# mpitid/babble

Hardware: AMD Instinct MI355X
Metric: consensus-ordered events/sec at N participants (higher is better)
Workload: dtype int32; 1 GPU; random-gossip DAG, 256 participants, 10000000 events per GPU, RunConsensus every K=256 events (39063 calls); participants=256, events_per_graph=10000000, k=256, graphs_per_gpu=1, parallelism=replicas1

## Files before the change

babble_amd/csrc/hge_engine.hip:

```cpp
#include <hip/hip_runtime.h>

#include <algorithm>
#include <chrono>
#include <cstdio>
#include <cstdlib>
#include <cstring>
#include <mutex>
#include <optional>
#include <string>
#include <thread>
#include <utility>
#include <vector>

#include "../../include/hge.h"
#include "hge_plan.h"
#include "hge_kernels.hip"
#include "hge_median_rows.hip"
#include "hge_wide32.hip"
#include "hge_coords.hip"
#include "hge_coords_win.hip"
#include "hge_rounds_coop.hip"
#include "hge_rounds_direct.hip"
#include "hge_walk_spec.hip"

// ... 1346 lines not shown
    if (getenv("HGE_WALK_DEBUG")) {
      std::vector<int32_t> hn(2 * nw);
      std::vector<uint64_t> mg(nw);
      readback(hn.data(), s_cn.p, hn.size());
      readback(mg.data(), s_cM.p, mg.size());
      fprintf(stderr, "coop walk: nw=%d Hcap=%d resume=%d |", nw, Hcap, hres[1]);
      for (int i = 0; i < nw; i++)
        fprintf(stderr, " %d:%d%s->(%d,w%d:%d)", i, hn[i], hn[nw + i] ? "e" : "",
                mg[i] == ~0ull ? -1 : (int)(mg[i] >> 32),
                mg[i] == ~0ull ? -1 : i + (int)((mg[i] >> 16) & 0xFFFF), (int)(mg[i] & 0xFFFF));
      fprintf(stderr, "\n");
    }
    return hres[1];
  }
  void wide_walk(Tables t, const CoordStep& s, int32_t rlo, const int32_t* rlo_dev, int Rprev) {
    const int32_t* FDT = d_FDT.p;
    const int32_t* olen = s.olen;
    const int32_t* len = s.len;
    int32_t* rstate = s.rstate;
    int32_t* err = s_bar.p + 1;
    uint64_t* gran = s_gran.p;
    uint64_t* ssc = d_ssc.p;
    uint64_t* dbg = dbg_p();
    if (direct_rounds()) {
      uint32_t* mb = walk_mb();
      unsigned long long* paths = walk_paths();
      unsigned long long* paths_next = s_wpaths.p + 2 * ((walk_seq + 1) & 1);
      const int32_t* nostart = nullptr;
      int32_t* nohist = nullptr;
      int hmax = 0, extra = 0;
      const char* hs = getenv("HGE_TEST_HANDOFF_STALL");
      int stall_ep = hs ? atoi(hs) : 0;
      int force_exact = walk_force_exact();
      void* dargs[] = {&t, &olen, &len, &rstate, &rlo, &rlo_dev, &Rprev, &gran, &err, &ssc, &mb, &dbg,
                       &nostart, &nohist, &hmax, &nostart, &extra, &stall_ep, &force_exact, &paths, &paths_next};
      prof_begin("k_rounds_direct");
      HIPCHK(launch_resident(direct_fn(), dim3(N), dim3(1024), dargs));
      prof_end();
    } else {
      void* args[] = {&t, &FDT, &olen, &len, &rstate, &rlo, &rlo_dev, &Rprev, &gran, &err, &ssc, &dbg};
      prof_begin("k_rounds_coop");
      HIPCHK(launch_resident((const void*)k_rounds_coop, dim3(N), dim3(COOP_BS), args));
      prof_end();
    }
    if (getenv("HGE_TEST_HANDOFF_FAIL")) {
      const int32_t one = 1, down = hge_plan::kRoundsStoodDown;
      h2d(err, &one, 4);
      h2d(rstate + 1, &down, 4);
    }
  }
  uint32_t* walk_mb() {
    s_mb.need((size_t)npow() * npow());
    return s_mb.p;
  }
  DBuf<unsigned long long> s_wpaths;
  int walk_seq = 0;
  unsigned long long* walk_paths() {
    if (!s_wpaths.p) {
      s_wpaths.need(4);
      HIPCHK(hipMemset(s_wpaths.p, 0, 4 * sizeof(unsigned long long)));
    }
    walk_seq++;
    return s_wpaths.p + 2 * (walk_seq & 1);
  }
  static int walk_force_exact() {
    const char* e = getenv("HGE_TEST_DIR_EXACT");
    return e && atoi(e) != 0 ? 1 : 0;
  }
  const void* direct_fn() const {
    return N <= 64 ? (const void*)k_rounds_direct<1024, 64>
         : N <= 128 ? (const void*)k_rounds_direct<1024, 128>
                    : (const void*)k_rounds_direct<1024, 256>;
  }

  bool sweep16() const { return N > 32 && !wide32; }
  bool wla16() const { return N > 192 && (N & 3) == 0 && !wide32; }

  void to_wide32() {
    auto test_stop = [&](int stage) {
      if (test_w32_fail == stage) {
        test_w32_fail = 0;
        throw EngineError(HGE_ERR_DEVICE, "test: to_wide32 stopped after stage " + std::to_string(stage));
      }
    };
    ensure_fdtd();
// ... 1575 lines not shown
  const int N = h->N, NW = h->NW;
  h->s_hist.need((size_t)hmax * N + N);
  h->s_hssc.need((size_t)hmax * N * NW);
  h->s_hstate.need(N + 4);
  h->h2d(h->s_hstate.p, start, 4 * (size_t)N);
  int32_t* cut = nullptr;
  if (stopcut) {
    h->s_hist.need((size_t)hmax * N + 2 * N);
    cut = h->s_hist.p + (size_t)hmax * N + N;
    h->h2d(cut, stopcut, 4 * (size_t)N);
  }
  int32_t* rstate = h->s_hstate.p + N;
  HIPCHK(hipMemsetAsync(rstate, 0, 16, h->st));
  h->s_bar.need(2);
  h->s_gran.need(2 * (size_t)N);
  HIPCHK(hipMemsetAsync(h->s_bar.p, 0, 8, h->st));
  HIPCHK(hipMemsetAsync(h->s_gran.p, 0, 16 * (size_t)N, h->st));
  auto lk = h->frontier_lock();
  Tables t = h->tables();
  const int32_t* olen = h->cstep->olen;
  const int32_t* len = h->cstep->len;
  int rlo = 0, Rprev = 0;
  const int32_t* rlo_dev = nullptr;
  uint64_t* gran = h->s_gran.p;
  int32_t* err = h->s_bar.p + 1;
  uint64_t* ssc = h->s_hssc.p;
  uint32_t* mb = h->walk_mb();
  unsigned long long* paths = h->walk_paths();
  unsigned long long* paths_next = h->s_wpaths.p + 2 * ((h->walk_seq + 1) & 1);
  uint64_t* dbg = nullptr;
  const int32_t* st0 = h->s_hstate.p;
  int32_t* hist = h->s_hist.p;
  int hm = hmax, ex = std::max(0, (int)extra), nostall = 0, force_exact = hge_engine::walk_force_exact();
  void* args[] = {&t, &olen, &len, &rstate, &rlo, &rlo_dev, &Rprev, &gran, &err, &ssc, &mb, &dbg,
                  &st0, &hist, &hm, &cut, &ex, &nostall, &force_exact, &paths, &paths_next};
  h->prof_begin("k_rounds_direct_walk");
  HIPCHK(h->launch_resident(h->direct_fn(), dim3(N), dim3(1024), args));
  h->prof_end();
  int32_t rs[2] = {0, 0}, e = 0;
  h->d2h(rs, rstate, 8);
  h->d2h(&e, err, 4);
  h->sync();
  if (e) throw EngineError(HGE_ERR_DEVICE, "rounds frontier hand-off timed out");
  const int n = std::max(1, std::min(rs[0], hmax));
  if (rows_out) h->readback(rows_out, h->s_hist.p, (size_t)n * N);
  if (ssc_out) h->readback(ssc_out, h->s_hssc.p, (size_t)n * N * NW);
  if (nrows) *nrows = n;
  if (natural) *natural = rs[1] == 0 ? 1 : 0;
  return HGE_OK;
  GUARD_END(h)
}

int hge_frontier_rows(hge_engine* h, int32_t from, int32_t n, int32_t* rows_out, uint64_t* ssc_out) {
  GUARD_BEGIN
  const int N = h->N, NW = h->NW;
  if (from < 0 || n < 0 || (size_t)(from + n) * N > h->s_hist.n) return HGE_ERR_ARG;
  if (rows_out && n) h->d2h(rows_out, h->s_hist.p + (size_t)from * N, 4 * (size_t)n * N);
  if (ssc_out && n) h->d2h(ssc_out, h->s_hssc.p + (size_t)from * N * NW, 8 * (size_t)n * N * NW);
  h->sync();
  return HGE_OK;
  GUARD_END(h)
}

int hge_split_finish(hge_engine* h, const int32_t* rows, const uint64_t* ssc, int32_t nrows,
                     int32_t natural, int64_t* n_ordered) {
  GUARD_BEGIN
  if (!h->cstep || !rows || nrows < 1 || (nrows > 1 && !ssc)) return HGE_ERR_ARG;
  const int N = h->N, NW = h->NW;
// ... 541 lines not shown
```

babble_amd/csrc/hge_narrow.h:

```cpp
#pragma once

#include <stdint.h>

#if defined(__HIPCC__) || defined(__CUDACC__)
#define HGE_NAR_HD __host__ __device__ __forceinline__
#else
#define HGE_NAR_HD inline
#endif

namespace hge_narrow {

constexpr uint32_t kNarGuard = 0x80808080u;
constexpr uint32_t kNarAMax = 126;
constexpr uint32_t kNarBaseNone = 0xFFFEu;
constexpr int32_t kNarBaseMax = 65400;
constexpr int32_t kNarInf32 = 0x7FFFFFFF;

HGE_NAR_HD uint32_t nar_base16(int32_t P) { return P == kNarInf32 ? kNarBaseNone : (uint32_t)P; }
HGE_NAR_HD bool nar_base_too_large(int32_t P) { return P != kNarInf32 && P > kNarBaseMax; }

HGE_NAR_HD uint32_t nar_sub_sat2(uint32_t x, uint32_t c) {
#if defined(__HIP_DEVICE_COMPILE__)
  typedef unsigned short u16x2 __attribute__((ext_vector_type(2)));
  const u16x2 r = __builtin_elementwise_sub_sat(__builtin_bit_cast(u16x2, x), __builtin_bit_cast(u16x2, c));
// ... 19 lines not shown
  const u16x2 r = __builtin_elementwise_max(__builtin_bit_cast(u16x2, x), __builtin_bit_cast(u16x2, y));
  return __builtin_bit_cast(uint32_t, r);
#else
  const uint32_t xl = x & 0xFFFFu, yl = y & 0xFFFFu, xh = x >> 16, yh = y >> 16;
  return (xl > yl ? xl : yl) | ((xh > yh ? xh : yh) << 16);
#endif
}
HGE_NAR_HD uint32_t nar_pack4(uint32_t x0, uint32_t x1) {
#if defined(__HIP_DEVICE_COMPILE__)
  return __builtin_amdgcn_perm(x1, x0, 0x06040200u);
#else
  return (x0 & 0xFFu) | ((x0 >> 8) & 0xFF00u) | ((x1 & 0xFFu) << 16) | ((x1 << 8) & 0xFF000000u);
#endif
}

HGE_NAR_HD uint32_t nar_enc_window4(uint32_t la0, uint32_t la1, uint32_t c0, uint32_t c1, uint32_t& mx) {
  const uint32_t cap = kNarAMax | (kNarAMax << 16);
  const uint32_t x0 = nar_sub_sat2(la0, c0), x1 = nar_sub_sat2(la1, c1);
  mx = nar_max2(mx, nar_max2(x0, x1));
  return nar_pack4(nar_min2(x0, cap), nar_min2(x1, cap)) | kNarGuard;
}
HGE_NAR_HD bool nar_window_flag(uint32_t mx) { return (mx & 0xFFFFu) >= kNarAMax || (mx >> 16) >= kNarAMax; }

HGE_NAR_HD uint32_t nar_enc_member4(uint32_t fd0, uint32_t fd1, uint32_t c0, uint32_t c1, uint32_t& mn) {
  const uint32_t cap = kNarAMax | (kNarAMax << 16);
  const uint32_t t0 = nar_sub_sat2(fd0, c0), t1 = nar_sub_sat2(fd1, c1);
  mn = nar_min2(mn, nar_min2(t0, t1));
  return nar_pack4(nar_min2(t0, cap), nar_min2(t1, cap)) + 0x01010101u;
}
HGE_NAR_HD bool nar_member_flag(uint32_t mn) { return (mn & 0xFFFFu) == 0 || (mn >> 16) == 0; }

HGE_NAR_HD uint32_t nar_ge4(uint32_t aw, uint32_t bw) { return (aw - bw) & kNarGuard; }

}
```

babble_amd/csrc/hge_rounds_direct.hip:

```cpp
#include <hip/hip_runtime.h>
#include <stdint.h>

#include "hge_narrow.h"

#ifndef HGE_DIR_NARROW_64
#define HGE_DIR_NARROW_64 1
#endif
#ifndef HGE_DIR_NARROW_128
#define HGE_DIR_NARROW_128 1
#endif
#ifndef HGE_DIR_NARROW_256
#define HGE_DIR_NARROW_256 1
#endif

namespace hge {

#ifdef HGE_DIR_STAMPS
constexpr bool kDirStamps = true;
#else
constexpr bool kDirStamps = false;
#endif
constexpr int DIR_MAXP = 16;
constexpr int DIR_CH = 32;

// ... 4 lines not shown
  static constexpr int CPT = NPOW / TPM;
  static constexpr int CW = CPT / 2;
  static constexpr int VW = (CW % 4 == 0) ? 4 : 2;
  static constexpr int PS = CW + VW;
  static constexpr int RS = TPM * PS;
  static constexpr int WIN_INTS = W * NPOW;
  static constexpr int PREF = (DIR_CH * NPOW / 4 + BS - 1) / BS;
  static constexpr int MBW = NPOW / 2;
  static constexpr int MVW = (CW % 4 == 0) ? 4 : 2;
  static constexpr bool NARROW = NPOW <= 64 ? HGE_DIR_NARROW_64 != 0
                               : NPOW <= 128 ? HGE_DIR_NARROW_128 != 0 : HGE_DIR_NARROW_256 != 0;
  static constexpr int H = W / 2;
  static constexpr int NCW = CW / 2;
  static constexpr int NVW = (NCW % 4 == 0) ? 4 : (NCW % 2 == 0) ? 2 : 1;
  static constexpr int NPS = NCW + NVW;
  static constexpr int NRS = TPM * NPS;
  static constexpr int NENC = (H * NPOW / 4 + BS - 1) / BS;
};

__device__ __forceinline__ int dir_tid() {
  int x = threadIdx.x;
  asm volatile("" : "+v"(x));
  return x;
}

template <int BS, int NPOW>
struct DirLDS {
  int sP[256];
  uint32_t sLA[DirGeo<BS, NPOW>::W * DirGeo<BS, NPOW>::RS] __attribute__((aligned(16)));
  int sCnt[DIR_MAXP];
  int sCntW[DIR_MAXP][BS / 64] __attribute__((aligned(16)));
  int sHist[DirGeo<BS, NPOW>::W / 2];
  uint32_t sBits[8];
  uint32_t sB16[DirGeo<BS, NPOW>::NARROW ? DirGeo<BS, NPOW>::RS : 4] __attribute__((aligned(16)));
  uint32_t sN[DirGeo<BS, NPOW>::NARROW ? DirGeo<BS, NPOW>::H * DirGeo<BS, NPOW>::NRS : 4] __attribute__((aligned(16)));
  int sEx[2];
  int sFlag[2];
  int s_stamp;
  uint64_t sdbg[2];
};

__device__ __forceinline__ uint32_t dir_pack_la(int a, int b) {
  return (uint32_t)(a + 2) | ((uint32_t)(b + 2) << 16);
}
__device__ __forceinline__ uint32_t dir_pack_fd(int a, int b) {
  const uint32_t lo = a == INF32 ? 0xFFFFu : (uint32_t)(a + 1);
  const uint32_t hi = b == INF32 ? 0xFFFFu : (uint32_t)(b + 1);
  return lo | (hi << 16);
}

template <int BS, int NPOW>
__device__ __forceinline__ void dir_fetch(const Tables& t, int c, int p0, int nr, int lenc,
                                          uint2 (&v)[DirGeo<BS, NPOW>::PREF]) {
  using G = DirGeo<BS, NPOW>;
  const int N = t.N;
  nr = min(nr, DIR_CH);
  const int have = (p0 == INF32 || nr <= 0) ? 0 : max(0, min(nr, lenc - p0));
  if (have == 0) return;
  const uint32_t* base = t.LA16 + ((size_t)c * t.ccap + p0) * (size_t)t.NW2;
  const int qmax = have * N / 4 - 1;
  const int tx = dir_tid();
#pragma unroll
  for (int m = 0; m < G::PREF; m++) {
    const int q = min(tx + m * BS, qmax);
    v[m] = *(const uint2*)(base + 2 * (size_t)q);
  }
}

template <int BS, int NPOW>
// ... 54 lines not shown
    if (!act || c0 + 4 * k >= N) a = make_int4(INF32, INF32, INF32, INF32);
    mw[2 * k] = dir_pack_fd(a.x, a.y);
    mw[2 * k + 1] = dir_pack_fd(a.z, a.w);
  }
}

template <int BS, int NPOW>
__device__ __forceinline__ void dir_members_mb(const uint32_t* mb, uint32_t (&mw)[DirGeo<BS, NPOW>::CW]) {
  using G = DirGeo<BS, NPOW>;
  constexpr int MVW = G::MVW;
  const __amdgpu_buffer_rsrc_t rs =
      __builtin_amdgcn_make_buffer_rsrc((void*)mb, 0, BS * G::CW * 4, 0x00020000);
  const int tx = dir_tid();
#pragma unroll
  for (int k = 0; k < G::CW / MVW; k++) {
    const int off = (k * BS + tx) * MVW * 4;
    if constexpr (MVW == 4) {
      typedef uint32_t u32x4 __attribute__((ext_vector_type(4)));
      const u32x4 x = __builtin_amdgcn_raw_buffer_load_b128(rs, off, 0, 16);
      mw[4 * k] = x.x;
      mw[4 * k + 1] = x.y;
      mw[4 * k + 2] = x.z;
      mw[4 * k + 3] = x.w;
    } else {
      typedef uint32_t u32x2 __attribute__((ext_vector_type(2)));
      const u32x2 x = __builtin_amdgcn_raw_buffer_load_b64(rs, off, 0, 16);
      mw[2 * k] = x.x;
      mw[2 * k + 1] = x.y;
    }
  }
}

template <int BS, int NPOW>
__device__ __forceinline__ void dir_stage_member(const Tables& t, uint32_t* mb, int c, int p) {
  using G = DirGeo<BS, NPOW>;
  constexpr int MVW = G::MVW;
  int lane = threadIdx.x;
  asm volatile("" : "+v"(lane));
  const int N = t.N;
  if (4 * lane < NPOW) {
    unsigned long long x;
    if (t.FD16) {
      uint2 a = make_uint2(~0u, ~0u);
      if (p != INF32 && 4 * lane < N) a = *(const uint2*)(t.FD16 + rowoff(t, c, p) + 4 * lane);
      x = (unsigned long long)a.x | ((unsigned long long)a.y << 32);
    } else {
      int4 a = make_int4(INF32, INF32, INF32, INF32);
      if (p != INF32 && 4 * lane < N) a = *(const int4*)(t.FD + rowoff(t, c, p) + 4 * lane);
      x = (unsigned long long)dir_pack_fd(a.x, a.y) | ((unsigned long long)dir_pack_fd(a.z, a.w) << 32);
    }
    const int w = 2 * lane, part = w / G::CW, wp = w - part * G::CW;
    const int k = wp / MVW, sub = wp - k * MVW;
    const size_t word = ((size_t)k * BS + (size_t)c * G::TPM + part) * MVW + sub;
    __hip_atomic_store((gu64_t*)(mb + word), x, __ATOMIC_RELAXED, __HIP_MEMORY_SCOPE_AGENT);
  }
}

template <int BS, int NPOW>
__device__ __forceinline__ int dir_count(const DirLDS<BS, NPOW>& L, int p, int part,
                                         const uint32_t (&mw)[DirGeo<BS, NPOW>::CW]) {
  using G = DirGeo<BS, NPOW>;
  const uint32_t* src = L.sLA + (p & (DirGeo<BS, NPOW>::W - 1)) * G::RS + part * G::PS;
  uint32_t acc0 = 0, acc1 = 0;
  const uint32_t ones = 0x00010001u;
  static_assert(G::CW % 2 == 0, "member slices are whole word pairs");
  static_assert(G::CW % G::VW == 0, "LDS reads cover whole slices");
#pragma unroll
  for (int k0 = 0; k0 < G::CW; k0 += G::VW) {
    uint32_t la[G::VW];
    if constexpr (G::VW == 4) {
      const uint4 q = *(const uint4*)(src + k0);
      la[0] = q.x;
      la[1] = q.y;
      la[2] = q.z;
      la[3] = q.w;
    } else {
      const uint2 q = *(const uint2*)(src + k0);
      la[0] = q.x;
      la[1] = q.y;
    }
#pragma unroll
    for (int k = 0; k < G::VW; k += 2) {
      uint32_t d0, d1;
      asm("v_pk_sub_u16 %0, %4, %6 clamp\n\t"
          "v_pk_sub_u16 %1, %5, %7 clamp\n\t"
          "v_pk_min_u16 %0, %0, %8\n\t"
          "v_pk_min_u16 %1, %1, %8\n\t"
          "v_pk_add_u16 %2, %2, %0\n\t"
          "v_pk_add_u16 %3, %3, %1"
          : "=&v"(d0), "=&v"(d1), "+v"(acc0), "+v"(acc1)
          : "v"(la[k]), "v"(la[k + 1]), "v"(mw[k0 + k]), "v"(mw[k0 + k + 1]), "v"(ones));
    }
  }
  int cnt = (int)(acc0 & 0xFFFFu) + (int)(acc0 >> 16) + (int)(acc1 & 0xFFFFu) + (int)(acc1 >> 16);
  if constexpr (G::TPM > 1) cnt += __builtin_amdgcn_mov_dpp(cnt, 0xB1, 0xF, 0xF, false);
  if constexpr (G::TPM > 2) cnt += __builtin_amdgcn_mov_dpp(cnt, 0x4E, 0xF, 0xF, false);
  if constexpr (G::TPM > 4) cnt += __builtin_amdgcn_mov_dpp(cnt, 0x141, 0xF, 0xF, false);
  if constexpr (G::TPM > 8) cnt += __builtin_amdgcn_mov_dpp(cnt, 0x140, 0xF, 0xF, false);
  static_assert(G::TPM <= 16, "a member's lanes lie in one DPP row");
  return cnt;
}


template <int BS, int NPOW>
__device__ __forceinline__ int dir_base_slot(int d) {
  using G = DirGeo<BS, NPOW>;
  const int w = d >> 1, part = w / G::CW;
  return 2 * (part * G::PS + (w - part * G::CW)) + (d & 1);
}

template <int BS, int NPOW>
__device__ __forceinline__ uint32_t dir_encode_window(const Tables& t, DirLDS<BS, NPOW>& L, int lo) {
  using G = DirGeo<BS, NPOW>;
  constexpr int GPR = NPOW / 4;
  uint32_t mx = 0;
  const int tx = dir_tid();
#pragma unroll
  for (int m = 0; m < G::NENC; m++) {
    const int q = tx + m * BS;
    if (q >= G::H * GPR) continue;
    const int k = q / GPR, col = 4 * (q - k * GPR);
    const int part = col / G::CPT, cp = col - part * G::CPT;
    const int off = part * G::PS + cp / 2;
    uint32_t word = hge_narrow::kNarGuard;
    if (col < t.N) {
      const uint2 la = *(const uint2*)(L.sLA + ((lo + k) & (G::W - 1)) * G::RS + off);
      const uint2 cb = *(const uint2*)(L.sB16 + off);
      word = hge_narrow::nar_enc_window4(la.x, la.y, cb.x, cb.y, mx);
    }
    L.sN[k * G::NRS + part * G::NPS + cp / 4] = word;
  }
  return mx;
}

template <int BS, int NPOW>
__device__ __forceinline__ uint32_t dir_encode_members(const DirLDS<BS, NPOW>& L, int part,
                                                       const uint32_t (&mw)[DirGeo<BS, NPOW>::CW],
                                                       uint32_t (&nw)[DirGeo<BS, NPOW>::NCW]) {
  using G = DirGeo<BS, NPOW>;
  const uint32_t* src = L.sB16 + part * G::PS;
  uint32_t mn = 0xFFFFFFFFu;
#pragma unroll
  for (int k0 = 0; k0 < G::CW; k0 += G::VW) {
    uint32_t cb[G::VW];
    if constexpr (G::VW == 4) {
      const uint4 q = *(const uint4*)(src + k0);
      cb[0] = q.x;
      cb[1] = q.y;
      cb[2] = q.z;
      cb[3] = q.w;
    } else {
      const uint2 q = *(const uint2*)(src + k0);
      cb[0] = q.x;
      cb[1] = q.y;
    }
#pragma unroll
    for (int k = 0; k < G::VW; k += 2)
      nw[(k0 + k) / 2] = hge_narrow::nar_enc_member4(mw[k0 + k], mw[k0 + k + 1], cb[k], cb[k + 1], mn);
  }
  return mn;
}

template <int BS, int NPOW>
__device__ __forceinline__ int dir_count_n(const DirLDS<BS, NPOW>& L, int k, int part,
                                           const uint32_t (&nw)[DirGeo<BS, NPOW>::NCW]) {
  using G = DirGeo<BS, NPOW>;
  const uint32_t* src = L.sN + k * G::NRS + part * G::NPS;
  uint32_t acc0 = 0, acc1 = 0;
#pragma unroll
  for (int k0 = 0; k0 < G::NCW; k0 += G::NVW) {
    uint32_t a[G::NVW];
    if constexpr (G::NVW == 4) {
      const uint4 q = *(const uint4*)(src + k0);
// ... 153 lines not shown
  asm volatile("" : "+v"(lane));
  int v = lane < H ? L.sHist[lane] : 0;
  HGE_DPP_SCAN(v, dpp_add, 0);
  const uint64_t ge = __ballot(lane < H && v >= SM);
  const int ks = ge ? (int)__builtin_ctzll(ge) : H;
  if (ks < e) {
    pb = a <= ks;
    return lo + ks;
  }
  if constexpr (NAR) {
    if (lenc - lo <= H) {
      bool ps;
      if (dir_probe_n<BS, NPOW>(t, L, e, part, slot++, mw, ps) >= SM) {
        pb = ps;
        return lo + e;
      }
      return INF32;
    }
    uint32_t mx[DirGeo<BS, NPOW>::CW];
    dir_members_reload<BS, NPOW>(t, L, mb, first, d, part, mx);
    return dir_probe_search<BS, NPOW>(t, c, lenc, L, part, mx, slot, pv, lo, pb, e);
  } else {
    return dir_probe_search<BS, NPOW>(t, c, lenc, L, part, mw, slot, pv, lo, pb, e);
  }
}

template <int BS, int NPOW>
__global__ void __launch_bounds__(BS, 4) k_rounds_direct(Tables t, const int32_t* olen, const int32_t* len,
                                                      int32_t* rstate, int rlo, const int32_t* rlo_dev,
                                                      int Rprev, uint64_t* gran,
                                                      int32_t* err, uint64_t* ssc, uint32_t* mbuf,
                                                      uint64_t* dbg, const int32_t* start, int32_t* hist,
                                                      int hmax, const int32_t* stopcut, int extra, int stall_ep,
                                                      int force_exact, unsigned long long* paths,
                                                      unsigned long long* paths_next) {
  using G = DirGeo<BS, NPOW>;
  if (rlo_dev) {
    rlo = *rlo_dev;
    if (rlo == INF32) {
      if (blockIdx.x == 0 && threadIdx.x == 0 && paths) paths_next[0] = paths_next[1] = 0;
      return;
    }
  }
  uint64_t st_t = 0, st_acc[9] = {0, 0, 0, 0, 0, 0, 0, 0, 0};
  const bool stamping = kDirStamps && dbg && blockIdx.x == 0 && threadIdx.x == 0;
#define DSTAMP(k)                  \
  if (stamping) {                  \
    const uint64_t now_ = stamp(); \
    st_acc[(k)] += now_ - st_t;    \
    st_t = now_;                   \
  }
#define DSTAMP_START                \
  if (stamping) st_t = stamp();
  __shared__ DirLDS<BS, NPOW> L;
  const int N = t.N, NW = t.NW;
  const int c = blockIdx.x, tid = threadIdx.x;
  const int d = tid / G::TPM, part = tid - d * G::TPM;
  const int lenc = len[c];
  gu64_t* gr[2] = {(gu64_t*)gran, (gu64_t*)(gran + N)};
  uint32_t* mbp[2] = {mbuf, mbuf + (size_t)NPOW * G::MBW};
  if (tid < N) {
    int P;
    if (hist) {
      P = start[tid];
      if (c == 0) hist[tid] = P;
    } else {
      P = t.C[(size_t)rlo * N + tid];
      if (rlo == 0 && olen[tid] == 0 && len[tid] > 0) P = 0;
      if (c == 0 && rlo == 0 && olen[tid] == 0 && len[tid] > 0) t.C[tid] = 0;
    }
    L.sP[tid] = P;
  }
  if constexpr (G::NARROW) {
    if (tid < NPOW) ((uint16_t*)L.sB16)[dir_base_slot<BS, NPOW>(tid)] = tid < N ? (uint16_t)hge_narrow::nar_base16(L.sP[tid]) : 0;
  }
  if (tid == 0) {
    L.s_stamp = stamping ? 1 : 0;
    L.sdbg[0] = L.sdbg[1] = 0;
    L.sEx[0] = L.sEx[1] = 0;
  }
  __syncthreads();
  if constexpr (G::NARROW) {
    if (tid < N && hge_narrow::nar_base_too_large(L.sP[tid])) atomicOr(&L.sEx[rlo & 1], 1);
  }
  int n_nar = 0, n_ex = 0;
  const int rcap = hist ? hmax : t.Rcap;
  int extra_left = -1;
  uint2 pv[G::PREF];
  int lo = L.sP[c];
  dir_load<BS, NPOW>(t, L, c, lo, DirGeo<BS, NPOW>::W, lenc, pv);
  int f0 = INF32, fn = 0;
  uint32_t mw[G::CW];
  dir_members_fd<BS, NPOW>(t, d, part, d < N ? L.sP[d] : INF32, mw);
  if constexpr (G::NARROW) __syncthreads();
  for (int r = rlo;; r++) {
    if (r + 1 >= rcap) {
      if (c == 0 && tid == 0) {
        rstate[1] = 1;
        if (hist) rstate[0] = r + 1;
      }
      break;
    }
    DSTAMP_START
    if (d >= N) {
#pragma unroll
      for (int k = 0; k < G::CW; k++) mw[k] = 0xFFFFFFFFu;
    }
    if (tid < DIR_MAXP) L.sCnt[tid] = 0;
    if (tid < 8) L.sBits[tid] = 0;
    if (tid < DirGeo<BS, NPOW>::W / 2) L.sHist[tid] = 0;
    if (tid == 0) {
      L.sFlag[(r + 1) & 1] = 0;
      L.sEx[(r + 1) & 1] = 0;
    }
    const int Pc = L.sP[c];
    const int cur = (r + 1 < Rprev) ? t.C[(size_t)(r + 1) * N + c] : INF32;
    uint32_t nw[G::NCW];
    bool enc = false;
    if constexpr (G::NARROW) {
      enc = Pc != INF32 && cur == INF32 && lo != INF32 && lo < lenc && !force_exact;
      if (enc) {
        const uint32_t mx = dir_encode_window<BS, NPOW>(t, L, lo);
        const uint32_t mn = dir_encode_members<BS, NPOW>(L, part, mw, nw);
        if (hge_narrow::nar_window_flag(mx) || hge_narrow::nar_member_flag(mn)) L.sEx[r & 1] = 1;
      }
    }
    __syncthreads();
    DSTAMP(0);
    int slot = 0;
    int nxt = INF32;
    bool pb = false;
    const bool stall = stall_ep > 0 && r - rlo + 1 == stall_ep;
    auto publish = [&]() {
      DSTAMP(1);
      if (stamping) st_acc[6] += slot;
      if (tid < 64 && !(stall && c == 0)) {
        dir_stage_member<BS, NPOW>(t, mbp[(r + 1) & 1], c, nxt);
        asm volatile("s_waitcnt vmcnt(0)" ::: "memory");
        if (tid == 0) {
          if (hist) hist[(size_t)(r + 1) * N + c] = nxt;
          else if (nxt != INF32 && cur == INF32) t.C[(size_t)(r + 1) * N + c] = nxt;
          const uint64_t g = ((uint64_t)(uint32_t)(r - rlo + 1) << 32) | (uint32_t)nxt;
          __hip_atomic_store(gr[(r + 1) & 1] + c, (unsigned long long)g, __ATOMIC_RELAXED,
                             __HIP_MEMORY_SCOPE_AGENT);
        }
      }
    };
    if (Pc == INF32) {
      publish();
    } else if (cur != INF32) {
      nxt = cur;
      publish();
      if (nxt < lo || nxt >= lo + DirGeo<BS, NPOW>::W) {
        __syncthreads();
        lo = nxt;
        dir_load<BS, NPOW>(t, L, c, lo, DirGeo<BS, NPOW>::W, lenc, pv);
        __syncthreads();
      }
      pb = dir_count<BS, NPOW>(L, nxt, part, mw) >= t.SM;
    } else {
      int s;
      if constexpr (G::NARROW) {
        const uint32_t* mbr = mbp[r & 1];
        if (enc && L.sEx[r & 1] == 0) {
          n_nar++;
          s = dir_select<BS, NPOW, true>(t, c, lenc, L, d, part, nw, slot, pv, lo, pb, mbr, r == rlo);
        } else {
          n_ex++;
          dir_members_reload<BS, NPOW>(t, L, mbr, r == rlo, d, part, mw);
          s = dir_select<BS, NPOW, false>(t, c, lenc, L, d, part, mw, slot, pv, lo, pb, mbr, r == rlo);
        }
      } else {
        n_ex++;
        s = dir_select<BS, NPOW, false>(t, c, lenc, L, d, part, mw, slot, pv, lo, pb, nullptr, false);
      }
      nxt = s < lenc ? s : INF32;
      publish();
    }
    if (nxt != INF32) {
      if (part == 0 && d < N && pb) atomicOr(&L.sBits[d >> 5], 1u << (d & 31));
      __syncthreads();
      if (tid < NW)
        ssc[((size_t)(r + 1) * N + c) * NW + tid] =
            (uint64_t)L.sBits[2 * tid] | ((uint64_t)L.sBits[2 * tid + 1] << 32);
    }
    DSTAMP(2);
    if (nxt == INF32) {
      f0 = INF32;
      fn = 0;
    } else {
      f0 = (lo != INF32 && nxt < lo + DirGeo<BS, NPOW>::W) ? lo + DirGeo<BS, NPOW>::W : nxt;
      fn = nxt + DirGeo<BS, NPOW>::W - f0;
    }
    lo = nxt;
    dir_fetch<BS, NPOW>(t, c, f0, fn, lenc, pv);
    dir_store<BS, NPOW>(t, L, f0, fn, lenc, pv);
    if (fn > DIR_CH) {
      for (int q = DIR_CH; q < fn; q += DIR_CH) {
        dir_fetch<BS, NPOW>(t, c, f0 + q, fn - q, lenc, pv);
        dir_store<BS, NPOW>(t, L, f0 + q, fn - q, lenc, pv);
      }
    }
    asm volatile("s_waitcnt vmcnt(0)" ::: "memory");
    DSTAMP(3);
    {
      const int tp = dir_tid();
      const int d = tp / G::TPM, part = tp - d * G::TPM;
      const unsigned ep = (unsigned)(r - rlo + 1);
      const gu64_t* g = gr[(r + 1) & 1];
      unsigned spins = 0;
      bool fail = false;
      int P = INF32;
      for (;;) {
        bool ok = true;
        if (d < N) {
          const unsigned long long x = __hip_atomic_load(g + d, __ATOMIC_RELAXED, __HIP_MEMORY_SCOPE_AGENT);
          ok = (unsigned)(x >> 32) == ep;
          P = (int)(uint32_t)x;
        }
        if (__all(ok)) break;
        if (stall || ++spins > (1u << 21)) {
          fail = true;
          break;
        }
        __builtin_amdgcn_s_sleep(1);
      }
      __builtin_amdgcn_fence(__ATOMIC_ACQUIRE, "wavefront");
      if (part == 0 && d < N) {
        L.sP[d] = P;
        if constexpr (G::NARROW) ((uint16_t*)L.sB16)[dir_base_slot<BS, NPOW>(d)] = (uint16_t)hge_narrow::nar_base16(P);
      }
      if constexpr (G::NARROW) {
        if (__ballot(part == 0 && d < N && hge_narrow::nar_base_too_large(P)) != 0 && (threadIdx.x & 63) == 0)
          L.sEx[(r + 1) & 1] = 1;
      }
      const bool any = __ballot(d < N && P != INF32) != 0;
      const bool notpast = stopcut && __ballot(part == 0 && d < N && P < stopcut[d]) != 0;
      if ((threadIdx.x & 63) == 0 && (any || notpast || fail))
        atomicOr(&L.sFlag[(r + 1) & 1], (any ? 1 : 0) | (notpast ? 2 : 0) | (fail ? 4 : 0));
      if (fail && (threadIdx.x & 63) == 0) {
        atomicOr(err, 1);
        atomicOr(rstate + 1, 4);
      }
      if (!fail) {
        dir_members_mb<BS, NPOW>(mbp[(r + 1) & 1], mw);
      } else {
#pragma unroll
        for (int k = 0; k < G::CW; k++) mw[k] = 0;
      }
    }
    __syncthreads();
    DSTAMP(4);
    const int fl = L.sFlag[(r + 1) & 1];
    const int stop = (fl & 4) ? 2 : ((fl & 1) ? 0 : 1);
    if (stop) {
      if (stop == 1 && c == 0 && tid == 0) rstate[0] = hist ? r + 2 : max(rstate[0], r + 1);
      break;
    }
    if (stopcut) {
      if (extra_left < 0 && !(fl & 2)) extra_left = extra;
      if (extra_left >= 0 && extra_left-- == 0) {
        if (c == 0 && tid == 0) {
          rstate[0] = r + 2;
          rstate[1] = 2;
        }
        break;
      }
    }
  }
  if (tid == 0 && paths) {
    atomicAdd(paths, (unsigned long long)n_nar);
    atomicAdd(paths + 1, (unsigned long long)n_ex);
    if (c == 0) paths_next[0] = paths_next[1] = 0;
  }
  if (stamping) {
    for (int q = 0; q < 9; q++) dbg[q] += st_acc[q];
    dbg[9] += L.sdbg[0];
    dbg[10] += L.sdbg[1];
  }
#undef DSTAMP
#undef DSTAMP_START
}

template __global__ void k_rounds_direct<1024, 64>(Tables, const int32_t*, const int32_t*, int32_t*, int, const int32_t*, int,
    uint64_t*, int32_t*, uint64_t*, uint32_t*, uint64_t*, const int32_t*, int32_t*, int, const int32_t*, int, int, int, unsigned long long*, unsigned long long*);
template __global__ void k_rounds_direct<1024, 128>(Tables, const int32_t*, const int32_t*, int32_t*, int, const int32_t*, int,
    uint64_t*, int32_t*, uint64_t*, uint32_t*, uint64_t*, const int32_t*, int32_t*, int, const int32_t*, int, int, int, unsigned long long*, unsigned long long*);
template __global__ void k_rounds_direct<1024, 256>(Tables, const int32_t*, const int32_t*, int32_t*, int, const int32_t*, int,
    uint64_t*, int32_t*, uint64_t*, uint32_t*, uint64_t*, const int32_t*, int32_t*, int, const int32_t*, int, int, int, unsigned long long*, unsigned long long*);

}
```

Measured before the change: 203.1 million events/s.

## Publish pre-encoded narrow member rows and encode windows off the critical path

```diff
diff --git a/babble_amd/csrc/hge_engine.hip b/babble_amd/csrc/hge_engine.hip
--- a/babble_amd/csrc/hge_engine.hip
+++ b/babble_amd/csrc/hge_engine.hip
@@ -1402,8 +1402,11 @@
       const char* hs = getenv("HGE_TEST_HANDOFF_STALL");
       int stall_ep = hs ? atoi(hs) : 0;
       int force_exact = walk_force_exact();
+      const char* mf = getenv("HGE_TEST_DIR_MEMBER_FLAG");
+      int mflag_ep = mf ? atoi(mf) : 0;
       void* dargs[] = {&t, &olen, &len, &rstate, &rlo, &rlo_dev, &Rprev, &gran, &err, &ssc, &mb, &dbg,
-                       &nostart, &nohist, &hmax, &nostart, &extra, &stall_ep, &force_exact, &paths, &paths_next};
+                       &nostart, &nohist, &hmax, &nostart, &extra, &stall_ep, &force_exact, &mflag_ep, &paths,
+                       &paths_next};
       prof_begin("k_rounds_direct");
       HIPCHK(launch_resident(direct_fn(), dim3(N), dim3(1024), dargs));
       prof_end();
@@ -1420,7 +1423,7 @@
     }
   }
   uint32_t* walk_mb() {
-    s_mb.need((size_t)npow() * npow());
+    s_mb.need((size_t)npow() * npow() + (size_t)npow() * npow() / 2);
     return s_mb.p;
   }
   DBuf<unsigned long long> s_wpaths;
@@ -3062,8 +3065,9 @@
   const int32_t* st0 = h->s_hstate.p;
   int32_t* hist = h->s_hist.p;
   int hm = hmax, ex = std::max(0, (int)extra), nostall = 0, force_exact = hge_engine::walk_force_exact();
+  int nomflag = 0;
   void* args[] = {&t, &olen, &len, &rstate, &rlo, &rlo_dev, &Rprev, &gran, &err, &ssc, &mb, &dbg,
-                  &st0, &hist, &hm, &cut, &ex, &nostall, &force_exact, &paths, &paths_next};
+                  &st0, &hist, &hm, &cut, &ex, &nostall, &force_exact, &nomflag, &paths, &paths_next};
   h->prof_begin("k_rounds_direct_walk");
   HIPCHK(h->launch_resident(h->direct_fn(), dim3(N), dim3(1024), args));
   h->prof_end();
diff --git a/babble_amd/csrc/hge_narrow.h b/babble_amd/csrc/hge_narrow.h
--- a/babble_amd/csrc/hge_narrow.h
+++ b/babble_amd/csrc/hge_narrow.h
@@ -75,4 +75,17 @@
 
 HGE_NAR_HD uint32_t nar_ge4(uint32_t aw, uint32_t bw) { return (aw - bw) & kNarGuard; }
 
+HGE_NAR_HD int nar_mb_ncw(int bs, int npow) { return npow / 4 / (bs / npow); }
+HGE_NAR_HD int nar_mb_vw(int bs, int npow) {
+  const int ncw = nar_mb_ncw(bs, npow);
+  return ncw % 4 == 0 ? 4 : ncw % 2 == 0 ? 2 : 1;
 }
+HGE_NAR_HD uint32_t nar_mb_word(int bs, int npow, int member, int cw) {
+  const int tpm = bs / npow, ncw = nar_mb_ncw(bs, npow), vw = nar_mb_vw(bs, npow);
+  const int part = cw / ncw, j = cw - part * ncw, k = j / vw;
+  return (uint32_t)((k * bs + member * tpm + part) * vw + (j - k * vw));
+}
+
+constexpr uint32_t kNarGranFlag = 0x80000000u;
+
+}
diff --git a/babble_amd/csrc/hge_rounds_direct.hip b/babble_amd/csrc/hge_rounds_direct.hip
--- a/babble_amd/csrc/hge_rounds_direct.hip
+++ b/babble_amd/csrc/hge_rounds_direct.hip
@@ -60,9 +60,10 @@
   int sCntW[DIR_MAXP][BS / 64] __attribute__((aligned(16)));
   int sHist[DirGeo<BS, NPOW>::W / 2];
   uint32_t sBits[8];
-  uint32_t sB16[DirGeo<BS, NPOW>::NARROW ? DirGeo<BS, NPOW>::RS : 4] __attribute__((aligned(16)));
+  uint32_t sB16[2][DirGeo<BS, NPOW>::NARROW ? DirGeo<BS, NPOW>::RS : 4] __attribute__((aligned(16)));
   uint32_t sN[DirGeo<BS, NPOW>::NARROW ? DirGeo<BS, NPOW>::H * DirGeo<BS, NPOW>::NRS : 4] __attribute__((aligned(16)));
   int sEx[2];
+  int sBig;
   int sFlag[2];
   int s_stamp;
   uint64_t sdbg[2];
@@ -183,28 +184,75 @@
 }
 
 template <int BS, int NPOW>
-__device__ __forceinline__ void dir_stage_member(const Tables& t, uint32_t* mb, int c, int p) {
+__device__ __forceinline__ void dir_members_nb(const uint32_t* nb, uint32_t (&nw)[DirGeo<BS, NPOW>::NCW]) {
+  using G = DirGeo<BS, NPOW>;
+  constexpr int NVW = G::NVW;
+  const __amdgpu_buffer_rsrc_t rs =
+      __builtin_amdgcn_make_buffer_rsrc((void*)nb, 0, BS * G::NCW * 4, 0x00020000);
+  const int tx = dir_tid();
+#pragma unroll
+  for (int k = 0; k < G::NCW / NVW; k++) {
+    const int off = (k * BS + tx) * NVW * 4;
+    if constexpr (NVW == 4) {
+      typedef uint32_t u32x4 __attribute__((ext_vector_type(4)));
+      const u32x4 x = __builtin_amdgcn_raw_buffer_load_b128(rs, off, 0, 16);
+      nw[4 * k] = x.x;
+      nw[4 * k + 1] = x.y;
+      nw[4 * k + 2] = x.z;
+      nw[4 * k + 3] = x.w;
+    } else if constexpr (NVW == 2) {
+      typedef uint32_t u32x2 __attribute__((ext_vector_type(2)));
+      const u32x2 x = __builtin_amdgcn_raw_buffer_load_b64(rs, off, 0, 16);
+      nw[2 * k] = x.x;
+      nw[2 * k + 1] = x.y;
+    } else {
+      nw[k] = __builtin_amdgcn_raw_buffer_load_b32(rs, off, 0, 16);
+    }
+  }
+}
+
+template <int BS, int NPOW>
+__device__ __forceinline__ bool dir_stage_member(const Tables& t, uint32_t* mb, uint32_t* nb, const uint32_t* bases,
+                                                 int c, int p) {
   using G = DirGeo<BS, NPOW>;
   constexpr int MVW = G::MVW;
   int lane = threadIdx.x;
   asm volatile("" : "+v"(lane));
   const int N = t.N;
-  if (4 * lane < NPOW) {
-    unsigned long long x;
+  const bool act = 4 * lane < NPOW;
+  uint2 a = make_uint2(~0u, ~0u);
+  if (act) {
     if (t.FD16) {
-      uint2 a = make_uint2(~0u, ~0u);
       if (p != INF32 && 4 * lane < N) a = *(const uint2*)(t.FD16 + rowoff(t, c, p) + 4 * lane);
-      x = (unsigned long long)a.x | ((unsigned long long)a.y << 32);
     } else {
-      int4 a = make_int4(INF32, INF32, INF32, INF32);
-      if (p != INF32 && 4 * lane < N) a = *(const int4*)(t.FD + rowoff(t, c, p) + 4 * lane);
-      x = (unsigned long long)dir_pack_fd(a.x, a.y) | ((unsigned long long)dir_pack_fd(a.z, a.w) << 32);
+      int4 f = make_int4(INF32, INF32, INF32, INF32);
+      if (p != INF32 && 4 * lane < N) f = *(const int4*)(t.FD + rowoff(t, c, p) + 4 * lane);
+      a = make_uint2(dir_pack_fd(f.x, f.y), dir_pack_fd(f.z, f.w));
     }
     const int w = 2 * lane, part = w / G::CW, wp = w - part * G::CW;
     const int k = wp / MVW, sub = wp - k * MVW;
     const size_t word = ((size_t)k * BS + (size_t)c * G::TPM + part) * MVW + sub;
+    const unsigned long long x = (unsigned long long)a.x | ((unsigned long long)a.y << 32);
     __hip_atomic_store((gu64_t*)(mb + word), x, __ATOMIC_RELAXED, __HIP_MEMORY_SCOPE_AGENT);
   }
+  if constexpr (G::NARROW) {
+    if (nb) {
+      uint32_t mn = 0xFFFFFFFFu, word = 0;
+      if (act) {
+        const int w = 2 * lane, part = w / G::CW;
+        const uint2 cb = *(const uint2*)(bases + part * G::PS + (w - part * G::CW));
+        word = hge_narrow::nar_enc_member4(a.x, a.y, cb.x, cb.y, mn);
+      }
+      const uint32_t odd = (uint32_t)__builtin_amdgcn_mov_dpp((int)word, 0xF5, 0xF, 0xF, false);
+      if (act && (lane & 1) == 0) {
+        const unsigned long long x = (unsigned long long)word | ((unsigned long long)odd << 32);
+        __hip_atomic_store((gu64_t*)(nb + hge_narrow::nar_mb_word(BS, NPOW, c, lane)), x, __ATOMIC_RELAXED,
+                           __HIP_MEMORY_SCOPE_AGENT);
+      }
+      return __ballot(act && hge_narrow::nar_member_flag(mn)) != 0;
+    }
+  }
+  return false;
 }
 
 template <int BS, int NPOW>
@@ -261,7 +309,8 @@
 }
 
 template <int BS, int NPOW>
-__device__ __forceinline__ uint32_t dir_encode_window(const Tables& t, DirLDS<BS, NPOW>& L, int lo) {
+__device__ __forceinline__ uint32_t dir_encode_window(const Tables& t, DirLDS<BS, NPOW>& L, const uint32_t* bases,
+                                                      int lo) {
   using G = DirGeo<BS, NPOW>;
   constexpr int GPR = NPOW / 4;
   uint32_t mx = 0;
@@ -276,7 +325,7 @@
     uint32_t word = hge_narrow::kNarGuard;
     if (col < t.N) {
       const uint2 la = *(const uint2*)(L.sLA + ((lo + k) & (G::W - 1)) * G::RS + off);
-      const uint2 cb = *(const uint2*)(L.sB16 + off);
+      const uint2 cb = *(const uint2*)(bases + off);
       word = hge_narrow::nar_enc_window4(la.x, la.y, cb.x, cb.y, mx);
     }
     L.sN[k * G::NRS + part * G::NPS + cp / 4] = word;
@@ -285,11 +334,11 @@
 }
 
 template <int BS, int NPOW>
-__device__ __forceinline__ uint32_t dir_encode_members(const DirLDS<BS, NPOW>& L, int part,
+__device__ __forceinline__ uint32_t dir_encode_members(const uint32_t* bases, int part,
                                                        const uint32_t (&mw)[DirGeo<BS, NPOW>::CW],
                                                        uint32_t (&nw)[DirGeo<BS, NPOW>::NCW]) {
   using G = DirGeo<BS, NPOW>;
-  const uint32_t* src = L.sB16 + part * G::PS;
+  const uint32_t* src = bases + part * G::PS;
   uint32_t mn = 0xFFFFFFFFu;
 #pragma unroll
   for (int k0 = 0; k0 < G::CW; k0 += G::VW) {
@@ -509,7 +558,7 @@
                                                       int32_t* err, uint64_t* ssc, uint32_t* mbuf,
                                                       uint64_t* dbg, const int32_t* start, int32_t* hist,
                                                       int hmax, const int32_t* stopcut, int extra, int stall_ep,
-                                                      int force_exact, unsigned long long* paths,
+                                                      int force_exact, int mflag_ep, unsigned long long* paths,
                                                       unsigned long long* paths_next) {
   using G = DirGeo<BS, NPOW>;
   if (rlo_dev) {
@@ -536,6 +585,11 @@
   const int lenc = len[c];
   gu64_t* gr[2] = {(gu64_t*)gran, (gu64_t*)(gran + N)};
   uint32_t* mbp[2] = {mbuf, mbuf + (size_t)NPOW * G::MBW};
+  uint32_t* nbp[2] = {nullptr, nullptr};
+  if constexpr (G::NARROW) {
+    nbp[0] = mbuf + 2 * (size_t)NPOW * G::MBW;
+    nbp[1] = nbp[0] + (size_t)NPOW * NPOW / 4;
+  }
   if (tid < N) {
     int P;
     if (hist) {
@@ -549,16 +603,24 @@
     L.sP[tid] = P;
   }
   if constexpr (G::NARROW) {
-    if (tid < NPOW) ((uint16_t*)L.sB16)[dir_base_slot<BS, NPOW>(tid)] = tid < N ? (uint16_t)hge_narrow::nar_base16(L.sP[tid]) : 0;
+    if (tid < NPOW) {
+      const uint16_t b = tid < N ? (uint16_t)hge_narrow::nar_base16(L.sP[tid]) : 0;
+      ((uint16_t*)L.sB16[0])[dir_base_slot<BS, NPOW>(tid)] = b;
+      ((uint16_t*)L.sB16[1])[dir_base_slot<BS, NPOW>(tid)] = b;
+    }
   }
   if (tid == 0) {
     L.s_stamp = stamping ? 1 : 0;
     L.sdbg[0] = L.sdbg[1] = 0;
     L.sEx[0] = L.sEx[1] = 0;
+    L.sBig = 0;
   }
   __syncthreads();
   if constexpr (G::NARROW) {
-    if (tid < N && hge_narrow::nar_base_too_large(L.sP[tid])) atomicOr(&L.sEx[rlo & 1], 1);
+    if (tid < N && hge_narrow::nar_base_too_large(L.sP[tid])) {
+      L.sEx[rlo & 1] = 1;
+      L.sBig = 1;
+    }
   }
   int n_nar = 0, n_ex = 0;
   const int rcap = hist ? hmax : t.Rcap;
@@ -567,9 +629,26 @@
   int lo = L.sP[c];
   dir_load<BS, NPOW>(t, L, c, lo, DirGeo<BS, NPOW>::W, lenc, pv);
   int f0 = INF32, fn = 0;
-  uint32_t mw[G::CW];
-  dir_members_fd<BS, NPOW>(t, d, part, d < N ? L.sP[d] : INF32, mw);
-  if constexpr (G::NARROW) __syncthreads();
+  uint32_t mw[G::NARROW ? 1 : G::CW];
+  uint32_t nw[G::NARROW ? G::NCW : 1];
+  bool nar = false;
+  if constexpr (G::NARROW) {
+    __syncthreads();
+    nar = lo != INF32 && lo < lenc && !force_exact;
+    if (nar) {
+      uint32_t m16[G::CW];
+      dir_members_fd<BS, NPOW>(t, d, part, d < N ? L.sP[d] : INF32, m16);
+      if (d >= N) {
+#pragma unroll
+        for (int k = 0; k < G::CW; k++) m16[k] = 0xFFFFFFFFu;
+      }
+      const uint32_t mx = dir_encode_window<BS, NPOW>(t, L, L.sB16[rlo & 1], lo);
+      const uint32_t mn = dir_encode_members<BS, NPOW>(L.sB16[rlo & 1], part, m16, nw);
+      if (hge_narrow::nar_window_flag(mx) || hge_narrow::nar_member_flag(mn)) L.sEx[rlo & 1] = 1;
+    }
+  } else {
+    dir_members_fd<BS, NPOW>(t, d, part, d < N ? L.sP[d] : INF32, mw);
+  }
   for (int r = rlo;; r++) {
     if (r + 1 >= rcap) {
       if (c == 0 && tid == 0) {
@@ -579,29 +658,26 @@
       break;
     }
     DSTAMP_START
-    if (d >= N) {
-#pragma unroll
-      for (int k = 0; k < G::CW; k++) mw[k] = 0xFFFFFFFFu;
+    if constexpr (G::NARROW) {
+      if (d >= N) {
+#pragma unroll
+        for (int k = 0; k < G::NCW; k++) nw[k] = 0x7F7F7F7Fu;
+      }
+    } else {
+      if (d >= N) {
+#pragma unroll
+        for (int k = 0; k < G::CW; k++) mw[k] = 0xFFFFFFFFu;
+      }
     }
     if (tid < DIR_MAXP) L.sCnt[tid] = 0;
     if (tid < 8) L.sBits[tid] = 0;
     if (tid < DirGeo<BS, NPOW>::W / 2) L.sHist[tid] = 0;
     if (tid == 0) {
       L.sFlag[(r + 1) & 1] = 0;
-      L.sEx[(r + 1) & 1] = 0;
+      L.sEx[(r + 1) & 1] = L.sBig;
     }
     const int Pc = L.sP[c];
     const int cur = (r + 1 < Rprev) ? t.C[(size_t)(r + 1) * N + c] : INF32;
-    uint32_t nw[G::NCW];
-    bool enc = false;
-    if constexpr (G::NARROW) {
-      enc = Pc != INF32 && cur == INF32 && lo != INF32 && lo < lenc && !force_exact;
-      if (enc) {
-        const uint32_t mx = dir_encode_window<BS, NPOW>(t, L, lo);
-        const uint32_t mn = dir_encode_members<BS, NPOW>(L, part, mw, nw);
-        if (hge_narrow::nar_window_flag(mx) || hge_narrow::nar_member_flag(mn)) L.sEx[r & 1] = 1;
-      }
-    }
     __syncthreads();
     DSTAMP(0);
     int slot = 0;
@@ -612,12 +688,14 @@
       DSTAMP(1);
       if (stamping) st_acc[6] += slot;
       if (tid < 64 && !(stall && c == 0)) {
-        dir_stage_member<BS, NPOW>(t, mbp[(r + 1) & 1], c, nxt);
+        bool mflag = dir_stage_member<BS, NPOW>(t, mbp[(r + 1) & 1], nbp[(r + 1) & 1], L.sB16[r & 1], c, nxt);
+        if (mflag_ep > 0 && c == 1 && r - rlo + 1 == mflag_ep) mflag = true;
         asm volatile("s_waitcnt vmcnt(0)" ::: "memory");
         if (tid == 0) {
           if (hist) hist[(size_t)(r + 1) * N + c] = nxt;
           else if (nxt != INF32 && cur == INF32) t.C[(size_t)(r + 1) * N + c] = nxt;
-          const uint64_t g = ((uint64_t)(uint32_t)(r - rlo + 1) << 32) | (uint32_t)nxt;
+          const uint32_t epw = (uint32_t)(r - rlo + 1) | (mflag ? hge_narrow::kNarGranFlag : 0u);
+          const uint64_t g = ((uint64_t)epw << 32) | (uint32_t)nxt;
           __hip_atomic_store(gr[(r + 1) & 1] + c, (unsigned long long)g, __ATOMIC_RELAXED,
                              __HIP_MEMORY_SCOPE_AGENT);
         }
@@ -627,25 +705,46 @@
       publish();
     } else if (cur != INF32) {
       nxt = cur;
-      publish();
-      if (nxt < lo || nxt >= lo + DirGeo<BS, NPOW>::W) {
-        __syncthreads();
-        lo = nxt;
-        dir_load<BS, NPOW>(t, L, c, lo, DirGeo<BS, NPOW>::W, lenc, pv);
-        __syncthreads();
-      }
-      pb = dir_count<BS, NPOW>(L, nxt, part, mw) >= t.SM;
+      if constexpr (G::NARROW) {
+        if (nar && L.sEx[r & 1] == 0 && nxt >= lo && nxt - lo < G::H) {
+          publish();
+          pb = dir_count_n<BS, NPOW>(L, nxt - lo, part, nw) >= t.SM;
+        } else {
+          uint32_t m16[G::CW];
+          dir_members_reload<BS, NPOW>(t, L, mbp[r & 1], r == rlo, d, part, m16);
+          asm volatile("s_waitcnt vmcnt(0)" ::: "memory");
+          __syncthreads();
+          publish();
+          if (nxt < lo || nxt >= lo + DirGeo<BS, NPOW>::W) {
+            __syncthreads();
+            lo = nxt;
+            dir_load<BS, NPOW>(t, L, c, lo, DirGeo<BS, NPOW>::W, lenc, pv);
+            __syncthreads();
+          }
+          pb = dir_count<BS, NPOW>(L, nxt, part, m16) >= t.SM;
+        }
+      } else {
+        publish();
+        if (nxt < lo || nxt >= lo + DirGeo<BS, NPOW>::W) {
+          __syncthreads();
+          lo = nxt;
+          dir_load<BS, NPOW>(t, L, c, lo, DirGeo<BS, NPOW>::W, lenc, pv);
+          __syncthreads();
+        }
+        pb = dir_count<BS, NPOW>(L, nxt, part, mw) >= t.SM;
+      }
     } else {
       int s;
       if constexpr (G::NARROW) {
         const uint32_t* mbr = mbp[r & 1];
-        if (enc && L.sEx[r & 1] == 0) {
+        if (nar && L.sEx[r & 1] == 0) {
           n_nar++;
           s = dir_select<BS, NPOW, true>(t, c, lenc, L, d, part, nw, slot, pv, lo, pb, mbr, r == rlo);
         } else {
           n_ex++;
-          dir_members_reload<BS, NPOW>(t, L, mbr, r == rlo, d, part, mw);
-          s = dir_select<BS, NPOW, false>(t, c, lenc, L, d, part, mw, slot, pv, lo, pb, mbr, r == rlo);
+          uint32_t m16[G::CW];
+          dir_members_reload<BS, NPOW>(t, L, mbr, r == rlo, d, part, m16);
+          s = dir_select<BS, NPOW, false>(t, c, lenc, L, d, part, m16, slot, pv, lo, pb, mbr, r == rlo);
         }
       } else {
         n_ex++;
@@ -669,13 +768,31 @@
       f0 = (lo != INF32 && nxt < lo + DirGeo<BS, NPOW>::W) ? lo + DirGeo<BS, NPOW>::W : nxt;
       fn = nxt + DirGeo<BS, NPOW>::W - f0;
     }
+    bool late = false;
+    if constexpr (G::NARROW) {
+      nar = nxt != INF32 && !force_exact;
+      late = nar && fn > DirGeo<BS, NPOW>::W - G::H;
+    }
     lo = nxt;
     dir_fetch<BS, NPOW>(t, c, f0, fn, lenc, pv);
+    if constexpr (G::NARROW) {
+      if (nar && !late) {
+        const uint32_t mx = dir_encode_window<BS, NPOW>(t, L, L.sB16[r & 1], nxt);
+        if (hge_narrow::nar_window_flag(mx)) L.sEx[(r + 1) & 1] = 1;
+      }
+    }
     dir_store<BS, NPOW>(t, L, f0, fn, lenc, pv);
     if (fn > DIR_CH) {
       for (int q = DIR_CH; q < fn; q += DIR_CH) {
         dir_fetch<BS, NPOW>(t, c, f0 + q, fn - q, lenc, pv);
         dir_store<BS, NPOW>(t, L, f0 + q, fn - q, lenc, pv);
+      }
+    }
+    if constexpr (G::NARROW) {
+      if (late) {
+        __syncthreads();
+        const uint32_t mx = dir_encode_window<BS, NPOW>(t, L, L.sB16[r & 1], nxt);
+        if (hge_narrow::nar_window_flag(mx)) L.sEx[(r + 1) & 1] = 1;
       }
     }
     asm volatile("s_waitcnt vmcnt(0)" ::: "memory");
@@ -686,13 +803,18 @@
       const unsigned ep = (unsigned)(r - rlo + 1);
       const gu64_t* g = gr[(r + 1) & 1];
       unsigned spins = 0;
-      bool fail = false;
+      bool fail = false, mflag = false;
       int P = INF32;
       for (;;) {
         bool ok = true;
         if (d < N) {
           const unsigned long long x = __hip_atomic_load(g + d, __ATOMIC_RELAXED, __HIP_MEMORY_SCOPE_AGENT);
-          ok = (unsigned)(x >> 32) == ep;
+          if constexpr (G::NARROW) {
+            ok = ((unsigned)(x >> 32) & ~hge_narrow::kNarGranFlag) == ep;
+            mflag = ((unsigned)(x >> 32) & hge_narrow::kNarGranFlag) != 0;
+          } else {
+            ok = (unsigned)(x >> 32) == ep;
+          }
           P = (int)(uint32_t)x;
         }
         if (__all(ok)) break;
@@ -705,11 +827,13 @@
       __builtin_amdgcn_fence(__ATOMIC_ACQUIRE, "wavefront");
       if (part == 0 && d < N) {
         L.sP[d] = P;
-        if constexpr (G::NARROW) ((uint16_t*)L.sB16)[dir_base_slot<BS, NPOW>(d)] = (uint16_t)hge_narrow::nar_base16(P);
+        if constexpr (G::NARROW)
+          ((uint16_t*)L.sB16[(r + 1) & 1])[dir_base_slot<BS, NPOW>(d)] = (uint16_t)hge_narrow::nar_base16(P);
       }
       if constexpr (G::NARROW) {
+        if (__ballot(d < N && mflag) != 0 && (threadIdx.x & 63) == 0) L.sEx[(r + 1) & 1] = 1;
         if (__ballot(part == 0 && d < N && hge_narrow::nar_base_too_large(P)) != 0 && (threadIdx.x & 63) == 0)
-          L.sEx[(r + 1) & 1] = 1;
+          L.sBig = 1;
       }
       const bool any = __ballot(d < N && P != INF32) != 0;
       const bool notpast = stopcut && __ballot(part == 0 && d < N && P < stopcut[d]) != 0;
@@ -719,11 +843,20 @@
         atomicOr(err, 1);
         atomicOr(rstate + 1, 4);
       }
-      if (!fail) {
-        dir_members_mb<BS, NPOW>(mbp[(r + 1) & 1], mw);
+      if constexpr (G::NARROW) {
+        if (!fail) {
+          dir_members_nb<BS, NPOW>(nbp[(r + 1) & 1], nw);
+        } else {
+#pragma unroll
+          for (int k = 0; k < G::NCW; k++) nw[k] = 0;
+        }
       } else {
-#pragma unroll
-        for (int k = 0; k < G::CW; k++) mw[k] = 0;
+        if (!fail) {
+          dir_members_mb<BS, NPOW>(mbp[(r + 1) & 1], mw);
+        } else {
+#pragma unroll
+          for (int k = 0; k < G::CW; k++) mw[k] = 0;
+        }
       }
     }
     __syncthreads();
@@ -760,10 +893,10 @@
 }
 
 template __global__ void k_rounds_direct<1024, 64>(Tables, const int32_t*, const int32_t*, int32_t*, int, const int32_t*, int,
-    uint64_t*, int32_t*, uint64_t*, uint32_t*, uint64_t*, const int32_t*, int32_t*, int, const int32_t*, int, int, int, unsigned long long*, unsigned long long*);
+    uint64_t*, int32_t*, uint64_t*, uint32_t*, uint64_t*, const int32_t*, int32_t*, int, const int32_t*, int, int, int, int, unsigned long long*, unsigned long long*);
 template __global__ void k_rounds_direct<1024, 128>(Tables, const int32_t*, const int32_t*, int32_t*, int, const int32_t*, int,
-    uint64_t*, int32_t*, uint64_t*, uint32_t*, uint64_t*, const int32_t*, int32_t*, int, const int32_t*, int, int, int, unsigned long long*, unsigned long long*);
+    uint64_t*, int32_t*, uint64_t*, uint32_t*, uint64_t*, const int32_t*, int32_t*, int, const int32_t*, int, int, int, int, unsigned long long*, unsigned long long*);
 template __global__ void k_rounds_direct<1024, 256>(Tables, const int32_t*, const int32_t*, int32_t*, int, const int32_t*, int,
-    uint64_t*, int32_t*, uint64_t*, uint32_t*, uint64_t*, const int32_t*, int32_t*, int, const int32_t*, int, int, int, unsigned long long*, unsigned long long*);
-
-}
+    uint64_t*, int32_t*, uint64_t*, uint32_t*, uint64_t*, const int32_t*, int32_t*, int, const int32_t*, int, int, int, int, unsigned long long*, unsigned long long*);
+
+}
```

After: 224.2 million events/s, median of 6. 10.4% higher.
